# gautam-sabnis/A-Divide-and-Conquer-Strategy-for-High-Dimensional-Bayesian-Factor-Models

Hardware: AMD Instinct MI355X
Metric: Gibbs iters/sec (node) at p=20k,n=1k,g=64; cov-assembly MFMA util % (higher is better)
Workload: dtype f64; 1 GPU; c3: p=19968 (P=312 x g=64), n=1000, K=30 (k=1920), rho=0.5, thin=5, burnin=0 (assembly in timed region), asm_batch=96; global_batch=1000, parallelism=shards64/gpus1

## Files before the change

a-divide-and-conquer-strategy-for-high-dimensional-bayesian-factor-models_amd/csrc/ypass.h:

```cpp
#pragma once
#include "dcfm_internal.h"
#include "linalg.h"

namespace dcfm {

#ifndef DCFM_WP_RING
#define DCFM_WP_RING 3
#endif
constexpr int WP_RING = DCFM_WP_RING;
#ifndef DCFM_WP_RING_WIDE
#define DCFM_WP_RING_WIDE 4
#endif
constexpr int WP_RING_WIDE = DCFM_WP_RING_WIDE;
#ifndef DCFM_WP_SKIP_PAD
#define DCFM_WP_SKIP_PAD 1
#endif
constexpr bool WP_SKIP_PAD = DCFM_WP_SKIP_PAD;
template <int KW, int MT, int R = (KW > KP ? WP_RING_WIDE : WP_RING), class Pre>
__device__ __forceinline__ void wpass_acc(const Dims &d, const double *__restrict__ Y, const double *__restrict__ Lam,
                                          const double *__restrict__ omega, int m, int i0, int kt, d4 (&acc)[MT][2],
                                          Pre &&pre) {
    const int lane = threadIdx.x & 63;
    const int r = lane & 15, q = lane >> 4;
    const double *Y0 = Y + ((size_t)m * d.NP + i0 + r) * d.PP + 2 * q;
    const double *Y1 = Y0 + (size_t)16 * (MT - 1) * d.PP;
    const double *L = Lam + (size_t)m * d.PP * KW + 32 * kt + 2 * r;
    const double *wp = omega + (size_t)m * d.PP + 2 * q;
#pragma unroll
    for (int a = 0; a < MT; ++a)
#pragma unroll
        for (int b = 0; b < 2; ++b) acc[a][b] = d4{0.0, 0.0, 0.0, 0.0};
    const int nch = WP_SKIP_PAD ? (d.P + 7) >> 3 : d.PP >> 3;
    d2 y0[R], y1[R], ww[R], l0[R], l1[R];
    auto load = [&](int t, int k) {
        const int j = 8 * t;
        y0[k] = *reinterpret_cast<const d2 *>(Y0 + j);
        if (MT == 2) y1[k] = *reinterpret_cast<const d2 *>(Y1 + j);
        ww[k] = *reinterpret_cast<const d2 *>(wp + j);
        l0[k] = *reinterpret_cast<const d2 *>(L + (size_t)(j + 2 * q) * KW);
        l1[k] = *reinterpret_cast<const d2 *>(L + (size_t)(j + 2 * q + 1) * KW);
    };
    d4 acc2[MT][2];
#pragma unroll
    for (int a = 0; a < MT; ++a)
#pragma unroll
        for (int b = 0; b < 2; ++b) acc2[a][b] = d4{0.0, 0.0, 0.0, 0.0};
    auto mma = [&](int k) {
        const double b00 = ww[k].x * l0[k].x, b01 = ww[k].x * l0[k].y;
        const double b10 = ww[k].y * l1[k].x, b11 = ww[k].y * l1[k].y;
        acc[0][0] = mfma16x16x4(b00, y0[k].x, acc[0][0]);
        acc[0][1] = mfma16x16x4(b01, y0[k].x, acc[0][1]);
        if (MT == 2) {
            acc[MT - 1][0] = mfma16x16x4(b00, y1[k].x, acc[MT - 1][0]);
            acc[MT - 1][1] = mfma16x16x4(b01, y1[k].x, acc[MT - 1][1]);
        }
        acc2[0][0] = mfma16x16x4(b10, y0[k].y, acc2[0][0]);
        acc2[0][1] = mfma16x16x4(b11, y0[k].y, acc2[0][1]);
        if (MT == 2) {
            acc2[MT - 1][0] = mfma16x16x4(b10, y1[k].y, acc2[MT - 1][0]);
            acc2[MT - 1][1] = mfma16x16x4(b11, y1[k].y, acc2[MT - 1][1]);
        }
    };
#pragma unroll
    for (int k = 0; k < R - 1; ++k)
        if (k < nch) load(k, k);
    pre();
    for (int t = 0; t < nch; t += R) {
#pragma unroll
        for (int k = 0; k < R; ++k) {
            if (t + k + R - 1 < nch) load(t + k + R - 1, (k + R - 1) % R);
            if (t + k < nch) mma(k);
        }
    }
#pragma unroll
    for (int a = 0; a < MT; ++a)
#pragma unroll
        for (int b = 0; b < 2; ++b) acc[a][b] += acc2[a][b];
}

template <int KW, int MT = 2>
__device__ __forceinline__ void wpass_tile(const Dims &d, const double *__restrict__ Y,
                                           const double *__restrict__ Lam, const double *__restrict__ omega,
                                           double *__restrict__ W, int w, int kt) {
    const int nrb = d.NP / (64 * MT);
    const int m = w / nrb, rb = w % nrb;
    const int wave = threadIdx.x >> 6, lane = threadIdx.x & 63;
    const int i0 = rb * 64 * MT + wave * 16 * MT;
    const int r = lane & 15, q = lane >> 4;
    d4 acc[MT][2];
    wpass_acc<KW, MT>(d, Y, Lam, omega, m, i0, kt, acc, [] {});
#pragma unroll
    for (int a = 0; a < MT; ++a) {
        double *Wt = W + ((size_t)m * d.NP + i0 + 16 * a + r) * KW + 32 * kt + 2 * q;
#pragma unroll
        for (int g = 0; g < 4; ++g) {
            d2 v;
            v.x = acc[a][0][g];
            v.y = acc[a][1][g];
            *reinterpret_cast<d2 *>(Wt + 8 * g) = v;
        }
    }
}

template <int KW, bool IS_E, bool SAME_T, bool PS = false>
__device__ __forceinline__ void cpass_wave(const Dims &d, const double *__restrict__ Yp,
                                           const double *__restrict__ Xp,
                                           const double *__restrict__ Zp,
                                           const double *__restrict__ Xa,
                                           const double *__restrict__ Za, int s0, int nsw,
                                           int q, d4 (&acc)[2][2], int par = 0) {
    constexpr bool EXTRA = IS_E && !SAME_T, ETA = KW > KP;
    d2 yA[4], xA[4], zA[4], yB[4], xB[4], zB[4];
    auto load = [&](int s, d2 (&y)[4], d2 (&x)[4], d2 (&z)[4]) {
#pragma unroll
        for (int u = 0; u < 4; ++u) {
            const int i = 4 * (s + u) + q;
            x[u] = *reinterpret_cast<const d2 *>(Xp + (size_t)i * KW);
            if (!ETA) z[u] = *reinterpret_cast<const d2 *>(Zp + (size_t)i * KW);
            if (!IS_E) {
                y[u] = *reinterpret_cast<const d2 *>(Yp + (size_t)i * d.PP);
            } else if (EXTRA) {
                const d2 xa = *reinterpret_cast<const d2 *>(Xa + (size_t)i * KW);
                if (ETA) {
                    y[u] = xa;
                } else {
                    const d2 za = *reinterpret_cast<const d2 *>(Za + (size_t)i * KW);
                    y[u].x = eta_of(d.sr, d.s1r, xa.x, za.x);
                    y[u].y = eta_of(d.sr, d.s1r, xa.y, za.y);
                }
            }
        }
    };
    auto mma = [&](d2 (&y)[4], d2 (&x)[4], d2 (&z)[4]) {
#pragma unroll
        for (int u = 0; u < 4; ++u) {
            const double e0 = ETA ? x[u].x : eta_of(d.sr, d.s1r, x[u].x, z[u].x);
            const double e1 = ETA ? x[u].y : eta_of(d.sr, d.s1r, x[u].y, z[u].y);
            const double a0 = (IS_E && SAME_T) ? e0 : y[u].x, a1 = (IS_E && SAME_T) ? e1 : y[u].y;
            if constexpr (PS) {
                const double ep = par ? e1 : e0;
                acc[0][0] = mfma16x16x4(a0, ep, acc[0][0]);
                acc[1][0] = mfma16x16x4(a1, ep, acc[1][0]);
            } else {
                acc[0][0] = mfma16x16x4(a0, e0, acc[0][0]);
                acc[0][1] = mfma16x16x4(a0, e1, acc[0][1]);
                acc[1][0] = mfma16x16x4(a1, e0, acc[1][0]);
                acc[1][1] = mfma16x16x4(a1, e1, acc[1][1]);
            }
        }
    };
    const int nb = nsw >> 2;
    load(s0, yA, xA, zA);
    for (int b = 0; b < nb; b += 2) {
        if (b + 1 < nb) load(s0 + 4 * (b + 1), yB, xB, zB);
        mma(yA, xA, zA);
        if (b + 2 < nb) load(s0 + 4 * (b + 2), yA, xA, zA);
        if (b + 1 < nb) mma(yB, xB, zB);
    }
}

}
```

Measured before the change: 5701 iter/s.

## Add deeper Y-load ring and SGPR-based addressing to C-pass inner loop

For the non-eta, non-E C-pass path, the double-buffered load/mma loop is replaced by a ring of CP_YRING Y batches in flight. X/Z loads and eta formation are decoupled and run one batch ahead, and sched_barriers fix the order. Base pointers are made wave-uniform via readfirstlane so loads use scalar bases plus 32-bit vector offsets. This aims to hide global-load latency and cut VGPR address arithmetic, at the cost of more registers and more complex tail handling.

```diff
diff --git a/a-divide-and-conquer-strategy-for-high-dimensional-bayesian-factor-models_amd/csrc/ypass.h b/a-divide-and-conquer-strategy-for-high-dimensional-bayesian-factor-models_amd/csrc/ypass.h
--- a/a-divide-and-conquer-strategy-for-high-dimensional-bayesian-factor-models_amd/csrc/ypass.h
+++ b/a-divide-and-conquer-strategy-for-high-dimensional-bayesian-factor-models_amd/csrc/ypass.h
@@ -16,6 +16,11 @@
 #define DCFM_WP_SKIP_PAD 1
 #endif
 constexpr bool WP_SKIP_PAD = DCFM_WP_SKIP_PAD;
+#ifndef DCFM_CP_YRING
+#define DCFM_CP_YRING 3
+#endif
+constexpr int CP_YRING = DCFM_CP_YRING;
+static_assert(CP_YRING >= 2, "the C pass's Y ring holds the batch that multiplies and one in flight");
 template <int KW, int MT, int R = (KW > KP ? WP_RING_WIDE : WP_RING), class Pre>
 __device__ __forceinline__ void wpass_acc(const Dims &d, const double *__restrict__ Y, const double *__restrict__ Lam,
                                           const double *__restrict__ omega, int m, int i0, int kt, d4 (&acc)[MT][2],
@@ -100,6 +105,20 @@
             *reinterpret_cast<d2 *>(Wt + 8 * g) = v;
         }
     }
+}
+
+__device__ __forceinline__ const char *uniform_ptr(const void *p) {
+    const uint64_t v = (uint64_t)p;
+    const uint32_t lo = __builtin_amdgcn_readfirstlane((uint32_t)v), hi = __builtin_amdgcn_readfirstlane((uint32_t)(v >> 32));
+    return (const char *)(((uint64_t)hi << 32) | lo);
+}
+__device__ __forceinline__ const char *sgpr_base(const char *p) {
+    asm volatile("" : "+s"(p));
+    return p;
+}
+__device__ __forceinline__ d2 load_d2_at(const char *base, uint32_t off) {
+    typedef const __attribute__((address_space(1))) char *gchar;
+    return *reinterpret_cast<const __attribute__((address_space(1))) d2 *>((gchar)base + off);
 }
 
 template <int KW, bool IS_E, bool SAME_T, bool PS = false>
@@ -150,6 +169,93 @@
         }
     };
     const int nb = nsw >> 2;
+    if constexpr (!ETA && !IS_E && !PS) {
+        constexpr int R = CP_YRING;
+        d2 yr[R][4], xv[4], zv[4];
+        double e0[4], e1[4];
+        const size_t yrow = (size_t)d.PP * 32;
+        const char *Yw = (const char *)Yp + s0 * yrow, *Xw = (const char *)Xp + (size_t)s0 * (KW * 32);
+        const char *Yu = uniform_ptr(Yw), *Xu = uniform_ptr(Xw), *Zu = uniform_ptr((const char *)Zp + (size_t)s0 * (KW * 32));
+        const uint32_t yo = (uint32_t)(Yw - Yu) + (uint32_t)q * (uint32_t)d.PP * 8u;
+        const uint32_t xo = (uint32_t)(Xw - Xu) + (uint32_t)q * (KW * 8u);
+        auto load_y = [&](int b, int k) {
+#pragma unroll
+            for (int u = 0; u < 4; ++u) yr[k][u] = load_d2_at(sgpr_base(Yu + (size_t)(4 * b + u) * yrow), yo);
+        };
+        auto load_xz = [&](int b) {
+            const char *xb = sgpr_base(Xu + (size_t)b * (KW * 128)), *zb = sgpr_base(Zu + (size_t)b * (KW * 128));
+#pragma unroll
+            for (int u = 0; u < 4; ++u) {
+                xv[u] = load_d2_at(xb + u * (KW * 32), xo);
+                zv[u] = load_d2_at(zb + u * (KW * 32), xo);
+            }
+            __builtin_amdgcn_sched_barrier(0);
+        };
+        auto form_eta = [&] {
+            __builtin_amdgcn_sched_barrier(0);
+#pragma unroll
+            for (int u = 0; u < 4; ++u) {
+                e0[u] = eta_of(d.sr, d.s1r, xv[u].x, zv[u].x);
+                e1[u] = eta_of(d.sr, d.s1r, xv[u].y, zv[u].y);
+            }
+            __builtin_amdgcn_sched_barrier(0);
+        };
+        auto mma_y = [&](int k) {
+            __builtin_amdgcn_sched_barrier(0);
+#pragma unroll
+            for (int u = 0; u < 4; ++u) {
+                acc[0][0] = mfma16x16x4(yr[k][u].x, e0[u], acc[0][0]);
+                acc[0][1] = mfma16x16x4(yr[k][u].x, e1[u], acc[0][1]);
+                acc[1][0] = mfma16x16x4(yr[k][u].y, e0[u], acc[1][0]);
+                acc[1][1] = mfma16x16x4(yr[k][u].y, e1[u], acc[1][1]);
+            }
+            __builtin_amdgcn_sched_barrier(0);
+        };
+        auto start = [&](int c) {
+            load_y(0, 0);
+            load_xz(0);
+            if (1 < c) load_y(1, 1 % R);
+            form_eta();
+            if (1 < c) load_xz(1);
+#pragma unroll
+            for (int k = 2; k < R; ++k)
+                if (k < c) load_y(k, k);
+        };
+        auto run = [&](int b, int c) {
+#pragma unroll
+            for (int j = 0; j < 2 * R - 1; ++j) {
+                if (j >= c) continue;
+                mma_y(j % R);
+                if (j + 1 < c) form_eta();
+                if (j + 2 < c) load_xz(b + j + 2);
+                if (j + R < c) load_y(b + j + R, j % R);
+            }
+        };
+        if (nb < R) {
+#pragma unroll
+            for (int c = 1; c < R; ++c)
+                if (nb == c) {
+                    start(c);
+                    run(0, c);
+                }
+            return;
+        }
+        start(R);
+        int b = 0;
+        for (; b + 2 * R <= nb; b += R) {
+#pragma unroll
+            for (int k = 0; k < R; ++k) {
+                mma_y(k);
+                form_eta();
+                load_xz(b + k + 2);
+                load_y(b + k + R, k);
+            }
+        }
+#pragma unroll
+        for (int c = R; c < 2 * R; ++c)
+            if (nb - b == c) run(b, c);
+        return;
+    }
     load(s0, yA, xA, zA);
     for (int b = 0; b < nb; b += 2) {
         if (b + 1 < nb) load(s0 + 4 * (b + 1), yB, xB, zB);
```

Result: no change. 5742 iter/s, median of 6 (+0.7%).
